# slimgroup/dfno

Measured on AMD Instinct MI355X. Metric: sec/batch, lower is better.
Workload: dtype fp32; 1 GPU; model=dfno-two-phase-3d, global_batch=1, t_in=1, t_out=30, width=20, num_blocks=4, parallelism=spatial-model-parallel 1x1x1x1x1x1, step=fwd+relative-Lp-loss+bwd+adam, spectral_weights=complex64

## Files before the change

### dfno_amd/csrc/bindings.cpp

```cpp
#include <torch/extension.h>

#include "kernels.h"

PYBIND11_MODULE(TORCH_EXTENSION_NAME, m) {
  m.doc() = "dfno_amd MI355X (gfx950) native kernels";
  m.def("channel_mix_fwd", &channel_mix_fwd,
        "fused channel linear + bias + gelu: returns (y, z)");
  m.def("channel_mix_fwd_t", &channel_mix_fwd_t,
        "transposed channel contraction (grad-x)");
  m.def("channel_mix_bwd_w", &channel_mix_bwd_w,
        "split-s grad-W (+grad-bias) reduction");
  m.def("linear_res_gelu_fwd", &linear_res_gelu_fwd,
        "fused y = gelu(W @ x + res): returns (y, z)");
  m.def("irfft_linear_res_gelu_fwd", &irfft_linear_res_gelu_fwd,
        "fused y = gelu(W @ x + pad_irfft(Yt)): returns (y, z)");
  m.def("gelu_fwd", &gelu_fwd, "exact gelu");
  m.def("gelu_bwd", &gelu_bwd, "gelu backward (gy, z) -> gz");
  m.def("add_gelu_fwd", &add_gelu_fwd, "fused residual add + gelu: returns (y, z)");
  m.def("proj_head_fwd", &proj_head_fwd, "fused linear->gelu->linear head");
  m.def("proj_head_bwd", &proj_head_bwd,
        "fused head backward: returns (gz3, gb3, gW4, gb4)");
  m.def("channel_mix_bwd_fused", &channel_mix_bwd_fused,
        "fused trunk mix backward: (gx, gW, gb, gz)");
  m.def("proj_head_bwd_fused", &proj_head_bwd_fused,
        "fully-fused flagship head backward: (gx, gW3, gb3, gW4, gb4)");
  m.def("lift_head_fwd", &lift_head_fwd, "fused time-lift + channel-lift + gelus");
  m.def("lift_head_bwd", &lift_head_bwd,
        "lift head backward: (gx, gW1, gb1, gW2, gb2)");
  m.def("adam_step_", &adam_step_, "fused Adam step (in-place)");
  m.def("adam_step_batch_", &adam_step_batch_, "fused Adam step over a tensor list");
  m.def("adam_step_batch_fp8_", &adam_step_batch_fp8_,
        "fused Adam step with in-kernel e4m3 requantization (delayed scaling)");
  m.def("dft_c2c", &dft_c2c, "truncated/padded complex DFT along a dim");
  m.def("dft_rfft_trunc", &dft_rfft_trunc, "real->kept-low-modes DFT (last dim)");
  m.def("dft_rfft_trunc_adj", &dft_rfft_trunc_adj, "adjoint of dft_rfft_trunc");
  m.def("dft_rfft_trunc_adj_acc", &dft_rfft_trunc_adj_acc,
        "adjoint of dft_rfft_trunc with fused accumulate addend");
  m.def("dft_pad_irfft", &dft_pad_irfft, "kept modes -> real inverse (last dim)");
  m.def("dft_pad_irfft_adj", &dft_pad_irfft_adj, "adjoint of dft_pad_irfft");
  m.def("dft_zt_fwd", &dft_zt_fwd,
        "fused truncated (z,t) 2-D analysis (real -> kept-mode c64)");
  m.def("dft_zt_inv", &dft_zt_inv,
        "fused padded (z,t) 2-D synthesis (kept-mode c64 -> real)");
  m.def("dft_pad_irfft_bf16", &dft_pad_irfft_bf16,
        "pad_irfft with bf16 output (bf16 compute config)");
  m.def("dft_rfft_trunc_adj_bf16", &dft_rfft_trunc_adj_bf16,
        "rfft_trunc adjoint with bf16 output");
  m.def("spectral_corner_fwd", &spectral_corner_fwd,
        "corner-block complex spectral contraction (accumulate into y box)");
  m.def("spectral_corner_bwd_x", &spectral_corner_bwd_x,
        "corner-block spectral contraction adjoint wrt x");
  m.def("spectral_corners_fwd", &spectral_corners_fwd,
        "all corner boxes in one launch");
  m.def("spectral_corners_bwd_x", &spectral_corners_bwd_x,
        "all corner boxes adjoint wrt x in one launch");
  m.def("spectral_corners_bwd_w", &spectral_corners_bwd_w,
// ... 20 lines not shown
```

### dfno_amd/csrc/epilogue.hip

```cpp

#include <hip/hip_runtime.h>
#include <torch/extension.h>
#include <ATen/hip/impl/HIPStreamMasqueradingAsCUDA.h>

#include <algorithm>
#include <vector>

#include "kernels.h"
#include "gelu_math.h"

namespace {

constexpr int kBlock = 256;

template <int IMAX, int VEC, int IT, int OT, int NT, int MT>
__global__ __launch_bounds__(kBlock) void irfft_mix_gelu_kernel(
    const float* __restrict__ x, const float* __restrict__ W,
    const float* __restrict__ Yt, const float* __restrict__ tw,
    float* __restrict__ y, float* __restrict__ z,
    int B, int I_, int O_, long L, int N_, int m_, int LT, float scale,
    bool write_z) {
  constexpr bool PIN = NT > 0;
  const int I = IT > 0 ? IT : I_;
  const int O = OT > 0 ? OT : O_;
  const int N = PIN ? NT : N_;
  const int m = PIN ? MT : m_;
  const int M2 = 2 * m;
  const long S = L * N;

  extern __shared__ __align__(16) char smem_raw[];
  float* Wl = reinterpret_cast<float*>(smem_raw);
  float* twl = Wl + (((size_t)O * I + 3) & ~(size_t)3);
  float* Yl = twl + (PIN ? 0 : (((size_t)N * M2 + 3) & ~(size_t)3));
  for (int k = threadIdx.x; k < O * I; k += kBlock) Wl[k] = W[k];
  if constexpr (!PIN)
    for (int k = threadIdx.x; k < N * M2; k += kBlock) twl[k] = tw[k];

  const int CPL = N / VEC;
  const int line = (int)threadIdx.x / CPL;
  const int t0 = ((int)threadIdx.x - line * CPL) * VEC;
  const bool role = line < LT;

  float twc[PIN ? VEC : 1][PIN ? MT : 1], tws[PIN ? VEC : 1][PIN ? MT : 1];
  if constexpr (PIN) {
#pragma unroll
    for (int v = 0; v < VEC; ++v) {
      const float* twj = tw + (size_t)(role ? t0 + v : 0) * M2;
#pragma unroll
      for (int k = 0; k < MT; ++k) {
        twc[v][k] = twj[2 * k];
        tws[v][k] = twj[2 * k + 1];
      }
    }
  }

  const long ntl = (L + LT - 1) / LT;
  for (long tile = blockIdx.x; tile < (long)B * ntl; tile += gridDim.x) {
    const int b = (int)(tile / ntl);
    const long l0 = (tile - (long)b * ntl) * LT;
    const int nl = (int)min((long)LT, L - l0);

    __syncthreads();
    const int run = nl * M2;
    if constexpr (PIN) {
      const int run4 = run / 4;
      for (int idx = threadIdx.x; idx < O * run4; idx += kBlock) {
        const int o = idx / run4;
        const int r4 = idx - o * run4;
        const int k = (r4 * 2) % MT;
        float4 v = *reinterpret_cast<const float4*>(
            Yt + (((long)b * O + o) * L + l0) * M2 + (long)r4 * 4);
        const bool e0 = (k == 0) || (2 * k == NT);
        const bool e1 = (2 * (k + 1) == NT);
        const float f0 = e0 ? scale : 2.0f * scale;
        const float f1 = e1 ? scale : 2.0f * scale;
        v.x = f0 * v.x; v.y = e0 ? 0.0f : f0 * v.y;
        v.z = f1 * v.z; v.w = e1 ? 0.0f : f1 * v.w;
        *reinterpret_cast<float4*>(Yl + (size_t)o * LT * M2 + (size_t)r4 * 4) = v;
      }
    } else {
      for (int idx = threadIdx.x; idx < O * run; idx += kBlock) {
        const int o = idx / run;
        const int r = idx - o * run;
        const int k = (r >> 1) % m;
        const bool edge = (k == 0) || (2 * k == N);
        const float f = edge ? scale : 2.0f * scale;
        float v = f * Yt[(((long)b * O + o) * L + l0) * M2 + r];
        if (edge && (r & 1)) v = 0.0f;
        Yl[(size_t)o * LT * M2 + r] = v;
      }
    }
    __syncthreads();

    if (!role || line >= nl) continue;

    const long s = (l0 + line) * N + t0;
    const float* xb = x + ((long)b * I) * S + s;
    float xr[IMAX][VEC];
#pragma unroll
    for (int i = 0; i < IMAX; ++i) {
      if (i < I) {
        if constexpr (VEC == 2) {
          const float2 v = *reinterpret_cast<const float2*>(xb + (long)i * S);
          xr[i][0] = v.x; xr[i][1] = v.y;
        } else {
#pragma unroll
          for (int v = 0; v < VEC; ++v) xr[i][v] = xb[(long)i * S + v];
        }
      }
    }

    float* yb = y + ((long)b * O) * S + s;
    float* zb = z + ((long)b * O) * S + s;
    const float* yline = Yl + (size_t)line * M2;
#pragma unroll 2
    for (int o = 0; o < (OT > 0 ? OT : 1 << 20); ++o) {
      if (OT == 0 && o >= O) break;
      float acc[VEC], syn[VEC];
#pragma unroll
      for (int v = 0; v < VEC; ++v) { acc[v] = 0.0f; syn[v] = 0.0f; }
#pragma unroll
// ... 1 lines not shown
        if (i < I) {
          const float wv = Wl[(size_t)o * I + i];
#pragma unroll
          for (int v = 0; v < VEC; ++v) acc[v] += wv * xr[i][v];
        }
      }
      const float* yo = yline + (size_t)o * LT * M2;
      if constexpr (PIN) {
        float yk[2 * MT];
#pragma unroll
        for (int q = 0; q < MT / 2; ++q) {
          const float4 v = *reinterpret_cast<const float4*>(yo + 4 * q);
          yk[4 * q] = v.x; yk[4 * q + 1] = v.y;
          yk[4 * q + 2] = v.z; yk[4 * q + 3] = v.w;
        }
#pragma unroll
        for (int k = 0; k < MT; ++k) {
#pragma unroll
          for (int v = 0; v < VEC; ++v)
            syn[v] += yk[2 * k] * twc[v][k] - yk[2 * k + 1] * tws[v][k];
        }
      } else {
        for (int k = 0; k < m; ++k) {
          const float yr_ = yo[2 * k], yi_ = yo[2 * k + 1];
#pragma unroll
          for (int v = 0; v < VEC; ++v) {
            const float* twj = twl + (size_t)(t0 + v) * M2;
            syn[v] += yr_ * twj[2 * k] - yi_ * twj[2 * k + 1];
          }
        }
      }
#pragma unroll
      for (int v = 0; v < VEC; ++v) acc[v] += syn[v];
      if constexpr (VEC == 2) {
        if (write_z)
          *reinterpret_cast<float2*>(zb + (long)o * S) =
              make_float2(acc[0], acc[1]);
        *reinterpret_cast<float2*>(yb + (long)o * S) =
            make_float2(dfno_gelu::gelu(acc[0]), dfno_gelu::gelu(acc[1]));
      } else {
#pragma unroll
        for (int v = 0; v < VEC; ++v) {
          if (write_z) zb[(long)o * S + v] = acc[v];
          yb[(long)o * S + v] = dfno_gelu::gelu(acc[v]);
        }
      }
    }
  }
}

}

std::vector<at::Tensor> irfft_linear_res_gelu_fwd(const at::Tensor& x,
                                                  const at::Tensor& W,
                                                  const at::Tensor& Yt,
                                                  int64_t n_out, bool need_z) {
  TORCH_CHECK(x.is_cuda() && x.is_contiguous() && x.scalar_type() == at::kFloat,
              "irfft_linear_res_gelu: x must be contiguous fp32 on GPU");
  TORCH_CHECK(W.is_cuda() && W.is_contiguous() && W.scalar_type() == at::kFloat,
              "irfft_linear_res_gelu: W must be contiguous fp32 on GPU");
  TORCH_CHECK(Yt.is_cuda() && Yt.is_contiguous() &&
              Yt.scalar_type() == at::kComplexFloat,
              "irfft_linear_res_gelu: Yt must be contiguous complex64 on GPU");
  TORCH_CHECK(x.dim() == 3 && W.dim() == 2 && Yt.dim() == 4,
              "irfft_linear_res_gelu: x [B,I,S], W [O,I], Yt [B,O,L,m]");
  const int B = (int)x.size(0), I = (int)x.size(1);
  const long S = x.size(2);
  const int O = (int)W.size(0);
  const long L = Yt.size(2);
  const int m = (int)Yt.size(3);
  const int N = (int)n_out;
  TORCH_CHECK((int)W.size(1) == I, "irfft_linear_res_gelu: W/I mismatch");
  TORCH_CHECK(Yt.size(0) == B && (int)Yt.size(1) == O && L * N == S,
              "irfft_linear_res_gelu: Yt shape mismatch");
  TORCH_CHECK(I >= 1 && I <= 32 && O >= 1 && O <= 64 && N >= 1 && N <= 64 &&
              m >= 1 && m <= 32 && m <= N / 2 + 1,
              "irfft_linear_res_gelu: needs I<=32, O<=64, N<=64, m<=min(32,N/2+1)");

  auto y = at::empty({B, O, S}, x.options());
  auto z = need_z ? at::empty({B, O, S}, x.options())
                  : at::empty({0}, x.options());
  if (x.numel() == 0) return {y, z};

  auto stream = at::hip::getCurrentHIPStreamMasqueradingAsCUDA().stream();
  auto tw = dfno_twiddle_table(N, m, false, x.options());
  const float scale = (float)(1.0 / (double)N);
  const float* xp = x.data_ptr<float>();
  const float* Wp = W.data_ptr<float>();
  const float* Yp = reinterpret_cast<const float*>(Yt.data_ptr());
  const float* twp = tw.data_ptr<float>();
  float* yp = y.data_ptr<float>();
  float* zp = need_z ? z.data_ptr<float>() : yp;

  auto pad4 = [](size_t n) { return (n + 3) & ~(size_t)3; };
  if (I == 20 && O == 20 && N == 30 && m == 8) {
    constexpr int LT = 17;
    const long ntiles = (long)B * ((L + LT - 1) / LT);
    const int grid = (int)std::min(ntiles, 256L * 8);
    const size_t smem = sizeof(float) * (pad4(400) + (size_t)20 * LT * 16);
    hipLaunchKernelGGL((irfft_mix_gelu_kernel<20, 2, 20, 20, 30, 8>),
                       dim3(grid), dim3(kBlock), smem, stream, xp, Wp, Yp, twp,
                       yp, zp, B, I, O, L, N, m, LT, scale, need_z);
  } else {
    int LT = kBlock / N;
    const size_t line_bytes = sizeof(float) * (size_t)O * 2 * m;
    LT = (int)std::max<size_t>(1, std::min<size_t>(LT, (32 * 1024) / line_bytes));
    const long ntiles = (long)B * ((L + LT - 1) / LT);
    const int grid = (int)std::min(ntiles, 256L * 8);
    const size_t smem = sizeof(float) * (pad4((size_t)O * I) +
                                         pad4((size_t)N * 2 * m) +
                                         (size_t)O * LT * 2 * m);
#define EPI_GENERIC(CAP)                                                       \
    hipLaunchKernelGGL((irfft_mix_gelu_kernel<CAP, 1, 0, 0, 0, 0>),            \
                       dim3(grid), dim3(kBlock), smem, stream, xp, Wp, Yp,     \
                       twp, yp, zp, B, I, O, L, N, m, LT, scale, need_z);
    if (I <= 8) { EPI_GENERIC(8) }
    else if (I <= 16) { EPI_GENERIC(16) }
    else if (I <= 24) { EPI_GENERIC(24) }
    else { EPI_GENERIC(32) }
#undef EPI_GENERIC
  }
  DFNO_CHECK_LAUNCH("irfft_linear_res_gelu");
  return {y, z};
}
```

### dfno_amd/csrc/kernels.h

```cpp
#pragma once

#include <torch/extension.h>
#define DFNO_CHECK_LAUNCH(what)                                            \
  do {                                                                     \
    hipError_t _e = hipGetLastError();                                     \
    TORCH_CHECK(_e == hipSuccess, what, " launch failed: ",                \
                hipGetErrorString(_e));                                    \
  } while (0)

#include <vector>

std::vector<at::Tensor> channel_mix_fwd(const at::Tensor& x, const at::Tensor& W,
                                        const at::Tensor& b, bool act);

at::Tensor channel_mix_fwd_t(const at::Tensor& gz, const at::Tensor& W);

std::vector<at::Tensor> linear_res_gelu_fwd(const at::Tensor& x, const at::Tensor& W,
                                            const at::Tensor& res);

std::vector<at::Tensor> irfft_linear_res_gelu_fwd(const at::Tensor& x,
                                                  const at::Tensor& W,
                                                  const at::Tensor& Yt,
                                                  int64_t n_out, bool need_z);

at::Tensor dfno_twiddle_table(int N, int m, bool analysis,
                              const at::TensorOptions& opt);

at::Tensor gelu_fwd(const at::Tensor& x);
at::Tensor gelu_bwd(const at::Tensor& gy, const at::Tensor& z);
std::vector<at::Tensor> add_gelu_fwd(const at::Tensor& a, const at::Tensor& b);

at::Tensor proj_head_fwd(const at::Tensor& x, const at::Tensor& W3,
                         const at::Tensor& b3, const at::Tensor& W4,
                         const at::Tensor& b4);
std::vector<at::Tensor> proj_head_bwd(const at::Tensor& gy, const at::Tensor& x,
                                      const at::Tensor& W3, const at::Tensor& b3,
                                      const at::Tensor& W4);
std::vector<at::Tensor> proj_head_bwd_fused(const at::Tensor& gy,
                                            const at::Tensor& x,
                                            const at::Tensor& W3,
                                            const at::Tensor& b3,
                                            const at::Tensor& W4);

std::vector<at::Tensor> channel_mix_bwd_w(const at::Tensor& gz, const at::Tensor& x,
                                          bool want_bias);

std::vector<at::Tensor> channel_mix_bwd_fused(const at::Tensor& gy,
                                              const at::Tensor& z,
                                              const at::Tensor& x,
                                              const at::Tensor& W,
                                              bool want_bias, bool want_gz);

at::Tensor lift_head_fwd(const at::Tensor& x, const at::Tensor& W1,
                         const at::Tensor& b1, const at::Tensor& W2,
                         const at::Tensor& b2);
std::vector<at::Tensor> lift_head_bwd(const at::Tensor& gy, const at::Tensor& x,
                                      const at::Tensor& W1, const at::Tensor& b1,
                                      const at::Tensor& W2, const at::Tensor& b2);

void adam_step_(at::Tensor& p, const at::Tensor& g, at::Tensor& m, at::Tensor& v,
                double lr, double beta1, double beta2, double eps,
                double weight_decay, int64_t step);
void adam_step_batch_(std::vector<at::Tensor> ps, std::vector<at::Tensor> gs,
                      std::vector<at::Tensor> ms, std::vector<at::Tensor> vs,
                      double lr, double beta1, double beta2, double eps,
                      double weight_decay, std::vector<int64_t> steps);
std::vector<int64_t> adam_step_batch_fp8_(
    std::vector<at::Tensor> ps, std::vector<at::Tensor> gs,
    std::vector<at::Tensor> ms, std::vector<at::Tensor> vs,
    double lr, double beta1, double beta2, double eps, double weight_decay,
    std::vector<int64_t> steps, std::vector<at::Tensor> qs,
    std::vector<at::Tensor> am_ins, std::vector<at::Tensor> am_outs);

at::Tensor dft_c2c(const at::Tensor& x, int64_t dim, int64_t n,
                   int64_t m_lo, int64_t m_hi, bool analysis, double scale);
at::Tensor dft_rfft_trunc(const at::Tensor& x, int64_t dim, int64_t m);
at::Tensor dft_rfft_trunc_adj(const at::Tensor& gy, int64_t dim, int64_t n);
at::Tensor dft_rfft_trunc_adj_acc(const at::Tensor& gy, int64_t dim, int64_t n,
                                  const at::Tensor& accum);
at::Tensor dft_pad_irfft(const at::Tensor& y, int64_t dim, int64_t n_out, int64_t m);
at::Tensor dft_pad_irfft_adj(const at::Tensor& gx, int64_t dim, int64_t m);
at::Tensor dft_zt_fwd(const at::Tensor& x, int64_t mz_lo, int64_t mz_hi,
                      int64_t mt, double scale, bool factors);
at::Tensor dft_zt_inv(const at::Tensor& y, int64_t Z, int64_t T,
// ... 45 lines not shown
```

### dfno_amd/csrc/mix_bwd.hip

```cpp

#include <hip/hip_runtime.h>
#include <hip/hip_bf16.h>
#include <torch/extension.h>
#include <ATen/hip/impl/HIPStreamMasqueradingAsCUDA.h>

#include "kernels.h"
#include "gelu_math.h"

namespace {

constexpr int kBlock = 256;

typedef float f32x4_mb __attribute__((ext_vector_type(4)));

__device__ __forceinline__ float mb_ld(const float* p) { return *p; }
__device__ __forceinline__ float mb_ld(const unsigned short* p) {
  return __uint_as_float(((unsigned int)*p) << 16);
}
__device__ __forceinline__ void mb_st(float* p, float v) { *p = v; }
__device__ __forceinline__ void mb_st(unsigned short* p, float v) {
  __hip_bfloat16 h = __float2bfloat16(v);
  *p = *reinterpret_cast<unsigned short*>(&h);
}

template <typename TIO, bool WG, int PH = 7, int TS = 64>
__global__ __launch_bounds__(kBlock, 4) void mix_bwd_fused_kernel(
    const TIO* __restrict__ gy, const TIO* __restrict__ z,
    const TIO* __restrict__ x, const float* __restrict__ W,
    TIO* __restrict__ gx, float* __restrict__ gW, float* __restrict__ gb,
    TIO* __restrict__ gzout, int B, long S) {
  constexpr int C = 20;
  constexpr int LD = TS + 4;
  extern __shared__ __align__(16) char smem_raw[];
  float* gzt = reinterpret_cast<float*>(smem_raw);
  float* xt = gzt + (size_t)C * LD;

  const int lane = (int)(threadIdx.x & 63);
  const int wave = (int)(threadIdx.x >> 6);
  const int l16 = lane & 15;
  const int kg = lane >> 4;

  f32x4_mb wacc;
  wacc = f32x4_mb{0.f, 0.f, 0.f, 0.f};

  const long stiles = (S + TS - 1) / TS;
  const long tend = (long)B * stiles;
  constexpr int NPF = (2 * C * TS + kBlock - 1) / kBlock;
  float pfa[NPF], pfb[NPF];
  auto prefetch = [&](long tt) {
    if (tt >= tend) return;
    const int b = (int)(tt / stiles);
    const long s0 = (tt % stiles) * TS;
    const int nv = (int)min((long)TS, S - s0);
#pragma unroll
    for (int q = 0; q < NPF; ++q) {
      const int r = (int)threadIdx.x + q * kBlock;
      const int row = r / TS;
      const int c = r - row * TS;
// ... 4 lines not shown
        } else {
          const long off = ((long)b * C + (row - C)) * S + s0 + c;
          a = mb_ld(gy + off);
          bb = mb_ld(z + off);
        }
      }
      pfa[q] = a;
      pfb[q] = bb;
    }
  };
  prefetch(blockIdx.x);

  for (long t = blockIdx.x; t < tend; t += gridDim.x) {
    const int b = (int)(t / stiles);
    const long s0 = (t % stiles) * TS;
    const int nv = (int)min((long)TS, S - s0);
    __syncthreads();
#pragma unroll
    for (int q = 0; q < NPF; ++q) {
      const int r = (int)threadIdx.x + q * kBlock;
      const int row = r / TS;
      const int c = r - row * TS;
      if (row < C) {
        xt[row * LD + c] = pfa[q];
      } else {
        const float gzv = pfa[q] * dfno_gelu::gelu_grad(pfb[q]);
        gzt[(row - C) * LD + c] = gzv;
        if (WG && c < nv)
          mb_st(gzout + ((long)b * C + (row - C)) * S + s0 + c, gzv);
      }
    }
    prefetch(t + gridDim.x);
    __syncthreads();
    if constexpr ((PH & 2) == 0 && (PH & 4) == 0) continue;
#pragma unroll
    for (int pp = 0; pp < ((PH & 2) ? (2 * (TS / 16)) / 4 : 0); ++pp) {
      const int p = wave + 4 * pp;
      const int mt = p / (TS / 16), nt = p % (TS / 16);
      const int m = mt * 16 + l16;
      const int n = nt * 16 + l16;
      const bool av = m < C;
      f32x4_mb c4 = {0.f, 0.f, 0.f, 0.f};
#pragma unroll
      for (int k = 0; k < C; k += 4) {
        const int ko = k + kg;
        const float a = av ? W[ko * C + m] : 0.f;
        const float bb = gzt[ko * LD + n];
        c4 = __builtin_amdgcn_mfma_f32_16x16x4f32(a, bb, c4, 0, 0, 0);
      }
      const long sc = s0 + nt * 16 + l16;
      if (sc < S) {
#pragma unroll
        for (int r = 0; r < 4; ++r) {
          const int i = mt * 16 + kg * 4 + r;
          if (i < C) mb_st(gx + ((long)b * C + i) * S + sc, c4[r]);
        }
      }
    }
    if constexpr ((PH & 4) != 0) {
      const int mt = wave >> 1, nt = wave & 1;
      const float* gr = gzt + (mt * 16 + l16) * LD;
      const int ncol = nt * 16 + l16;
      const float* xr = xt + ncol * LD;
      const bool av = (mt * 16 + l16) < C;
      const bool bx = ncol < C;
      const bool bones = ncol == C;
#pragma unroll 8
      for (int k = 0; k < TS; k += 4) {
        const float a = av ? gr[k + kg] : 0.f;
        const float bb = bx ? xr[k + kg] : (bones ? 1.f : 0.f);
        wacc = __builtin_amdgcn_mfma_f32_16x16x4f32(a, bb, wacc, 0, 0, 0);
      }
    }
  }

  {
    const int mt = wave >> 1, nt = wave & 1;
#pragma unroll
    for (int r = 0; r < 4; ++r) {
      const int o = mt * 16 + kg * 4 + r;
      const int n = nt * 16 + l16;
      const float v = wacc[r];
      if (o < C && v != 0.f) {
        if (n < C) atomicAdd(&gW[(size_t)o * C + n], v);
        else if (n == C && gb != nullptr) atomicAdd(&gb[o], v);
      }
    }
  }
}

}

std::vector<at::Tensor> channel_mix_bwd_fused(const at::Tensor& gy,
                                              const at::Tensor& z,
                                              const at::Tensor& x,
                                              const at::Tensor& W,
                                              bool want_bias, bool want_gz) {
  const bool bf16 = gy.scalar_type() == at::kBFloat16;
  TORCH_CHECK(gy.is_cuda() && gy.is_contiguous() && z.is_contiguous() &&
              x.is_contiguous() && W.is_contiguous() &&
              (bf16 || gy.scalar_type() == at::kFloat) &&
              x.scalar_type() == gy.scalar_type() &&
              z.scalar_type() == gy.scalar_type() &&
              W.scalar_type() == at::kFloat,
              "mix_bwd_fused: fp32/bf16 activations, fp32 W");
  int B = (int)x.size(0), I = (int)x.size(1);
  long S = x.size(2);
  int O = (int)W.size(0);
  TORCH_CHECK(I == 20 && O == 20, "mix_bwd_fused: trunk 20x20 only");
  TORCH_CHECK(gy.numel() == x.numel() && z.numel() == x.numel(),
              "mix_bwd_fused: shape mismatch");

  auto gx = at::empty({B, I, S}, x.options());
  auto fopt = x.options().dtype(at::kFloat);
  auto gW = at::zeros({O, I}, fopt);
  auto gb = want_bias ? at::zeros({O}, fopt) : at::empty({0}, fopt);
  auto gz = want_gz ? at::empty({B, O, S}, x.options())
                    : at::empty({0}, x.options());
  if (x.numel() == 0) return {gx, gW, gb, gz};

  auto stream = at::hip::getCurrentHIPStreamMasqueradingAsCUDA().stream();
  static const bool ts128 = []() {
    const char* e = getenv("DFNO_MIX_TS128");
    return e && e[0] == '1';
  }();
  const int TS = ts128 ? 128 : 64;
  size_t smem = sizeof(float) * 2 * 20 * (TS + 4);
  long stiles = (S + TS - 1) / TS;
  int grid = (int)std::min((long)B * stiles, 1024L);
  float* gbp = want_bias ? gb.data_ptr<float>() : nullptr;
  static const int ph = []() {
    const char* e = getenv("DFNO_MIX_PHASES");
    return e ? atoi(e) : 7;
  }();
#define MB_LAUNCH(TIO, WG, GZP) MB_LAUNCH_T(TIO, WG, GZP, 7, 64)
#define MB_LAUNCH_P(TIO, WG, GZP, PHV) MB_LAUNCH_T(TIO, WG, GZP, PHV, 64)
#define MB_LAUNCH_T(TIO, WG, GZP, PHV, TSV)                                  \
  hipLaunchKernelGGL((mix_bwd_fused_kernel<TIO, WG, PHV, TSV>), dim3(grid), \
                     dim3(kBlock), smem, stream,                             \
                     reinterpret_cast<const TIO*>(gy.data_ptr()),            \
                     reinterpret_cast<const TIO*>(z.data_ptr()),             \
                     reinterpret_cast<const TIO*>(x.data_ptr()),             \
                     W.data_ptr<float>(),                                    \
                     reinterpret_cast<TIO*>(gx.data_ptr()),                  \
                     gW.data_ptr<float>(), gbp, GZP, B, S)
  if (bf16) {
    auto gzp = want_gz ? reinterpret_cast<unsigned short*>(gz.data_ptr())
                       : nullptr;
    if (want_gz) MB_LAUNCH(unsigned short, true, gzp);
    else         MB_LAUNCH(unsigned short, false, nullptr);
  } else {
    auto gzp = want_gz ? reinterpret_cast<float*>(gz.data_ptr()) : nullptr;
    if (want_gz) {
      if (ts128) { MB_LAUNCH_T(float, true, gzp, 7, 128); }
      else if (ph == 1) { MB_LAUNCH_T(float, true, gzp, 1, 64); }
      else if (ph == 3) { MB_LAUNCH_T(float, true, gzp, 3, 64); }
      else if (ph == 5) { MB_LAUNCH_T(float, true, gzp, 5, 64); }
      else { MB_LAUNCH_T(float, true, gzp, 7, 64); }
    }
    else         MB_LAUNCH(float, false, nullptr);
  }
#undef MB_LAUNCH_T
#undef MB_LAUNCH_P
#undef MB_LAUNCH
  DFNO_CHECK_LAUNCH("mix_bwd_fused");
  return {gx, gW, gb, gz};
}
```

### dfno_amd/nn/block.py

```python

from __future__ import annotations

from typing import Dict, List, Tuple

import numpy as np
import torch
import torch.nn as nn

import os

from ..comm import (Repartition, _get_plan, repartition_complete,
                    repartition_issue)
from ..partition import Partition, compute_distribution_info
from ..ops import spectral_conv, add_gelu, linear_res_gelu, rfft_trunc, fft_trunc, pad_ifft, pad_irfft
from ..ops import irfft_linear_res_gelu, fused_epilogue_enabled, fused_epilogue_ok
from ..timing import comm_region
from .linear import BroadcastedLinear

__all__ = ["DistributedFNOBlock"]


class DistributedFNOBlock(nn.Module):

    def __init__(self, P_x: Partition, in_shape, modes,
# ... 234 lines not shown
        T = self.in_shape[-1]
        m = min(self.restrict_prefixes[self.dim_m[-1]], T // 2 + 1)
        if not fused_epilogue_ok(self.dtype, self.width, self.width, T, m):
            return False
        if len(self.dim_m) == 2:
            from ..ops.fft import zt_enabled
            if zt_enabled():
                return False
        return _get_plan(self.P_m, self.P_x, tuple(self.in_shape)).is_identity

    def _chunk_sizes(self, nch: int):
        w = self.width
        base, rem = divmod(w, nch)
        return [base + (1 if i < rem else 0) for i in range(nch)]

    @staticmethod
    def _with_c(shape, c):
        s = list(shape)
        s[1] = c
        return s

    def forward(self, x: torch.Tensor) -> torch.Tensor:
        self.dt_comm = 0.0

        x_in = x
        with comm_region() as r:
            W_res = self.linear.W_bcast(self.linear.W)
        self.linear.dt_comm = r.host_dt

        nch = self._pipeline_chunks()
        if nch > 1:
            y = self._forward_pipelined(x, nch)
        else:
            y, x_in, spectrum = self._forward_seq(x)
            if spectrum:
                T = self.in_shape[-1]
                return irfft_linear_res_gelu(
                    x_in, W_res, y, T // 2 + 1, T,
                    self.restrict_prefixes[self.dim_m[-1]])

        return linear_res_gelu(x_in, W_res, y)

    def _forward_seq(self, x: torch.Tensor):
        from ..ops.fft import (StashGradFn, new_stash_key, rfft_trunc_stash,
                               stash_fusable)

        saved: Dict[int, int] = {}
        x_orig = x
        with comm_region() as r:
            x = self.R1(x)
        self.dt_comm += r.host_dt

        x_epi = x_orig
        outermost = self.dim_m[-1]
        zt_stash = False
        if (x is x_orig and len(self.dim_m) == 2 and x.is_cuda
                and x.numel() > 0 and x.dtype == torch.float32
                and torch.is_grad_enabled() and x.requires_grad):
            from ..ops.fft import zt_enabled, zt_fwd, zt_native_ok
            z_dim = self.dim_m[0]
            mzl = self.restrict_prefixes[z_dim]
            mzh = self.restrict_suffixes.get(z_dim, 0)
            mt = self.restrict_prefixes[outermost]
            if zt_enabled() and zt_native_ok(x, mzl, mzh, mt):
                key = new_stash_key()
                saved[outermost] = x.shape[outermost] // 2 + 1
                saved[z_dim] = x.shape[z_dim]
                xm, tok = zt_fwd(x, mzl, mzh, mt, stash_key=key)
                x_epi = StashGradFn.apply(x_orig, tok, key)
                x = xm
                zt_stash = True
        if zt_stash:
            pass
        elif (x is x_orig
                and stash_fusable(x, outermost, self.restrict_prefixes[outermost])):
            key = new_stash_key()
            saved[outermost] = x.shape[outermost] // 2 + 1
            xm, tok = rfft_trunc_stash(x, outermost,
                                       self.restrict_prefixes[outermost], key)
            for dim in reversed(self.dim_m[:-1]):
                saved[dim] = xm.shape[dim]
                xm = fft_trunc(xm, dim, self.restrict_prefixes[dim],
                               self.restrict_suffixes.get(dim, 0))
            x_epi = StashGradFn.apply(x_orig, tok, key)
            x = xm
        else:
            x = self._fwd_m(x, saved)

        with comm_region() as r:
            x = self.R2(x)
        self.dt_comm += r.host_dt

        if x.numel() > 0:
            x = self._fwd_y(x, saved)
            y = spectral_conv(x, list(self.weights), self.corner_bounds,
                              self.width, fp8=self.spectral_fp8)
            y = self._inv_y(y, saved)
        else:
            y = x

        with comm_region() as r:
            y = self.R3(y)
        self.dt_comm += r.host_dt

        defer = (y.is_cuda and y.numel() > 0 and y.dtype == torch.complex64
                 and self._fuse_epilogue())
        y = self._inv_m(y, saved, defer_irfft=defer)
        if defer:
            return y, x_epi, True

        with comm_region() as r:
            y = self.R4(y)
        self.dt_comm += r.host_dt
        return y, x_epi, False

    def _forward_pipelined(self, x: torch.Tensor, nch: int) -> torch.Tensor:
        sizes = self._chunk_sizes(nch)
        saved: Dict[int, int] = {}

        xs = list(x.split(sizes, dim=1)) if x.numel() > 0 else [x] * nch

        with comm_region() as r:
            h1 = [repartition_issue(self.R1, xc.contiguous(),
                                    self._with_c(self.in_shape, c))
                  for xc, c in zip(xs, sizes)]
        self.dt_comm += r.host_dt

        h2 = []
        for h, c in zip(h1, sizes):
            with comm_region() as r:
                xc = repartition_complete(h)
            self.dt_comm += r.host_dt
            xc = self._fwd_m(xc, saved)
            with comm_region() as r:
                h2.append(repartition_issue(self.R2, xc,
                                            self._with_c(self.trunc_m_shape, c)))
            self.dt_comm += r.host_dt

        zs = []
        for h in h2:
            with comm_region() as r:
                xc = repartition_complete(h)
            self.dt_comm += r.host_dt
            zs.append(self._fwd_y(xc, saved))

        if all(z.numel() == 0 for z in zs):
            x = zs[0]
# ... 40 lines not shown
```

### dfno_amd/ops/epilogue.py

```python

from __future__ import annotations

import os

import torch

from .. import _ext
from .fft import pad_irfft
from .pointwise import linear_res_gelu

__all__ = ["irfft_linear_res_gelu", "fused_epilogue_enabled",
           "fused_epilogue_ok"]


def fused_epilogue_enabled() -> bool:
    return os.environ.get("DFNO_FUSED_EPILOGUE", "1") != "0"


def fused_epilogue_ok(dtype, I: int, O: int, n_out: int, m: int) -> bool:
    return (dtype == torch.float32 and 1 <= I <= 32 and 1 <= O <= 64
            and 1 <= n_out <= 64 and 1 <= m <= min(32, n_out // 2 + 1))


class _IrfftLinearResGeluFn(torch.autograd.Function):
    @staticmethod
    def forward(ctx, x, W, Yt, n_out):
        ext = _ext.get(required=True)
        B, I = x.shape[0], x.shape[1]
        O, m = W.shape[0], Yt.shape[-1]
        S = x.numel() // max(B * I, 1)
        x3 = x.reshape(B, I, S).contiguous()
        Y4 = Yt.reshape(B, O, S // n_out, m).contiguous()
        need_z = any(ctx.needs_input_grad[:3])
        Wc = W.contiguous()
        y3, z3 = ext.irfft_linear_res_gelu_fwd(x3, Wc, Y4, n_out, need_z)
        if need_z:
            ctx.save_for_backward(x3, Wc, z3)
        ctx.x_shape = tuple(x.shape)
        ctx.y_shape = tuple(Yt.shape)
        ctx.n_out = n_out
        return y3

    @staticmethod
    def backward(ctx, gy):
        ext = _ext.get(required=True)
        x3, W, z3 = ctx.saved_tensors
        gy = gy.contiguous()
        B, I, S = x3.shape
        O = W.shape[0]
        m = ctx.y_shape[-1]
        if I == 20 and O == 20:
            gx, gW, _, gz = ext.channel_mix_bwd_fused(gy, z3, x3, W,
                                                      False, True)
        else:
            gz = ext.gelu_bwd(gy, z3)
            gx = ext.channel_mix_fwd_t(gz, W)
            gW, _ = ext.channel_mix_bwd_w(gz, x3, False)
        gY = ext.dft_pad_irfft_adj(gz.reshape(B, O, S // ctx.n_out, ctx.n_out),
                                   3, m)
        return (gx.reshape(ctx.x_shape), gW.to(W.dtype),
                gY.reshape(ctx.y_shape), None)


def irfft_linear_res_gelu(x: torch.Tensor, W: torch.Tensor, Yt: torch.Tensor,
                          n_half: int, n_out: int, m: int) -> torch.Tensor:
    m = min(m, n_half)
    if (x.is_cuda and x.numel() > 0 and Yt.dtype == torch.complex64
            and Yt.shape[-1] == m and x.shape[-1] == n_out
            and fused_epilogue_ok(x.dtype, x.shape[1], W.shape[0], n_out, m)):
        out = _IrfftLinearResGeluFn.apply(x, W, Yt, n_out)
        shape = list(x.shape)
        shape[1] = W.shape[0]
        return out.reshape(shape)
    res = pad_irfft(Yt, -1, n_half, n_out, m, out_dtype=x.dtype)
    if res.dtype != x.dtype:
        res = res.to(x.dtype)
    return linear_res_gelu(x, W, res)
```

### dfno_amd/ops/fft.py

```python

from __future__ import annotations

import os

import torch

from .. import _ext
from ..dispatch import note_fallback

__all__ = ["rfft_trunc", "fft_trunc", "pad_ifft", "pad_irfft"]

_MAX_N = 256


def _native_ok(x: torch.Tensor, n: int, m: int, op: str) -> bool:
    if not x.is_cuda:
        return False
    ok = (n <= _MAX_N and m <= 32
          and x.dtype in (torch.float32, torch.complex64,
                          torch.float64, torch.complex128))
    if not ok:
        note_fallback(op, f"N={n} (cap {_MAX_N}) / m={m} (cap 32) / "
                      f"dtype {x.dtype} outside the native-DFT range")
    return ok
# ... 116 lines not shown


class StashGradFn(torch.autograd.Function):

    @staticmethod
    def forward(ctx, x, tok, key):
        ctx.key = key
        return x.view_as(x)

    @staticmethod
    def backward(ctx, g):
        _GRAD_STASH[ctx.key] = g.contiguous()
        return None, torch.empty(0, device=g.device), None


class _RfftTruncStashFn(torch.autograd.Function):
    @staticmethod
    def forward(ctx, x, dim, m, key):
        ext = _ext.get(required=True)
        ctx.dim, ctx.m, ctx.n, ctx.key = dim, m, x.shape[dim], key
        ctx.bf16 = x.dtype == torch.bfloat16
        y = ext.dft_rfft_trunc(x.contiguous(), dim, m)
        tok = torch.empty(0, device=x.device)
        return y, tok

    @staticmethod
    def backward(ctx, gy, gtok):
        ext = _ext.get(required=True)
        acc = _GRAD_STASH.pop(ctx.key, None)
        if acc is None:
            raise RuntimeError(
                "rfft stash: epilogue gradient missing (stash backward did "
                "not run before the rfft adjoint)")
        if ctx.bf16:
            gx = ext.dft_rfft_trunc_adj_bf16(gy.contiguous(), ctx.dim,
                                             ctx.n, acc)
        else:
            gx = ext.dft_rfft_trunc_adj_acc(gy.contiguous(), ctx.dim,
                                            ctx.n, acc)
        return gx, None, None, None


def rfft_trunc_stash(x, dim, m, key):
    d = dim % x.dim()
    m = min(m, x.shape[d] // 2 + 1)
    return _RfftTruncStashFn.apply(x, d, m, key)


def stash_fusable(x, dim, m) -> bool:
    d = dim % x.dim()
    m = min(m, x.shape[d] // 2 + 1)
    if not (d == x.dim() - 1 and x.is_cuda and x.numel() > 0
            and torch.is_grad_enabled() and x.requires_grad
            and x.shape[d] <= _MAX_N and m <= 32):
        return False
    if x.dtype == torch.bfloat16:
        return rfft_bf16_native_ok(x, d, m)
    return x.dtype in (torch.float32, torch.float64)



_ZT_EMPTY = {}


def _zt_empty(device):
    t = _ZT_EMPTY.get(device)
    if t is None:
# ... 129 lines not shown
```

Baseline: 20.14 ms.

## Fuse rfft adjoint with W^T·gz grad-x in the spectral epilogue backward

The epilogue backward now skips computing grad-x inside the fused mix-backward kernel and instead stashes (gz, W). The rfft-truncation adjoint then computes gx = W^T gz + rfft_adj(G) in one kernel, reusing the irfft-mix kernel template in an adjoint mode that loads a transposed W and skips the Hermitian scaling. This removes a separate grad-x write and read plus an accumulate pass. The cost is more coupling through the grad stash and a kernel variant that depends on the twiddle-table and transposition conventions being right.

```diff
diff --git a/dfno_amd/csrc/bindings.cpp b/dfno_amd/csrc/bindings.cpp
--- a/dfno_amd/csrc/bindings.cpp
+++ b/dfno_amd/csrc/bindings.cpp
@@ -14,6 +14,8 @@
         "fused y = gelu(W @ x + res): returns (y, z)");
   m.def("irfft_linear_res_gelu_fwd", &irfft_linear_res_gelu_fwd,
         "fused y = gelu(W @ x + pad_irfft(Yt)): returns (y, z)");
+  m.def("rfft_adj_mix", &rfft_adj_mix,
+        "fused gx = W^T @ gz + rfft_trunc_adj(G, n)");
   m.def("gelu_fwd", &gelu_fwd, "exact gelu");
   m.def("gelu_bwd", &gelu_bwd, "gelu backward (gy, z) -> gz");
   m.def("add_gelu_fwd", &add_gelu_fwd, "fused residual add + gelu: returns (y, z)");
@@ -21,7 +23,9 @@
   m.def("proj_head_bwd", &proj_head_bwd,
         "fused head backward: returns (gz3, gb3, gW4, gb4)");
   m.def("channel_mix_bwd_fused", &channel_mix_bwd_fused,
-        "fused trunk mix backward: (gx, gW, gb, gz)");
+        "fused trunk mix backward: (gx, gW, gb, gz)",
+        py::arg("gy"), py::arg("z"), py::arg("x"), py::arg("W"),
+        py::arg("want_bias"), py::arg("want_gz"), py::arg("want_gx") = true);
   m.def("proj_head_bwd_fused", &proj_head_bwd_fused,
         "fully-fused flagship head backward: (gx, gW3, gb3, gW4, gb4)");
   m.def("lift_head_fwd", &lift_head_fwd, "fused time-lift + channel-lift + gelus");
diff --git a/dfno_amd/csrc/epilogue.hip b/dfno_amd/csrc/epilogue.hip
--- a/dfno_amd/csrc/epilogue.hip
+++ b/dfno_amd/csrc/epilogue.hip
@@ -13,7 +13,7 @@
 
 constexpr int kBlock = 256;
 
-template <int IMAX, int VEC, int IT, int OT, int NT, int MT>
+template <int IMAX, int VEC, int IT, int OT, int NT, int MT, bool ADJ = false>
 __global__ __launch_bounds__(kBlock) void irfft_mix_gelu_kernel(
     const float* __restrict__ x, const float* __restrict__ W,
     const float* __restrict__ Yt, const float* __restrict__ tw,
@@ -32,7 +32,14 @@
   float* Wl = reinterpret_cast<float*>(smem_raw);
   float* twl = Wl + (((size_t)O * I + 3) & ~(size_t)3);
   float* Yl = twl + (PIN ? 0 : (((size_t)N * M2 + 3) & ~(size_t)3));
-  for (int k = threadIdx.x; k < O * I; k += kBlock) Wl[k] = W[k];
+  if constexpr (ADJ) {
+    for (int k = threadIdx.x; k < O * I; k += kBlock) {
+      const int o = k / I;
+      Wl[k] = W[(size_t)(k - o * I) * O + o];
+    }
+  } else {
+    for (int k = threadIdx.x; k < O * I; k += kBlock) Wl[k] = W[k];
+  }
   if constexpr (!PIN)
     for (int k = threadIdx.x; k < N * M2; k += kBlock) twl[k] = tw[k];
 
@@ -67,26 +74,31 @@
       for (int idx = threadIdx.x; idx < O * run4; idx += kBlock) {
         const int o = idx / run4;
         const int r4 = idx - o * run4;
-        const int k = (r4 * 2) % MT;
         float4 v = *reinterpret_cast<const float4*>(
             Yt + (((long)b * O + o) * L + l0) * M2 + (long)r4 * 4);
-        const bool e0 = (k == 0) || (2 * k == NT);
-        const bool e1 = (2 * (k + 1) == NT);
-        const float f0 = e0 ? scale : 2.0f * scale;
-        const float f1 = e1 ? scale : 2.0f * scale;
-        v.x = f0 * v.x; v.y = e0 ? 0.0f : f0 * v.y;
-        v.z = f1 * v.z; v.w = e1 ? 0.0f : f1 * v.w;
+        if constexpr (!ADJ) {
+          const int k = (r4 * 2) % MT;
+          const bool e0 = (k == 0) || (2 * k == NT);
+          const bool e1 = (2 * (k + 1) == NT);
+          const float f0 = e0 ? scale : 2.0f * scale;
+          const float f1 = e1 ? scale : 2.0f * scale;
+          v.x = f0 * v.x; v.y = e0 ? 0.0f : f0 * v.y;
+          v.z = f1 * v.z; v.w = e1 ? 0.0f : f1 * v.w;
+        }
         *reinterpret_cast<float4*>(Yl + (size_t)o * LT * M2 + (size_t)r4 * 4) = v;
       }
     } else {
       for (int idx = threadIdx.x; idx < O * run; idx += kBlock) {
         const int o = idx / run;
         const int r = idx - o * run;
-        const int k = (r >> 1) % m;
-        const bool edge = (k == 0) || (2 * k == N);
-        const float f = edge ? scale : 2.0f * scale;
-        float v = f * Yt[(((long)b * O + o) * L + l0) * M2 + r];
-        if (edge && (r & 1)) v = 0.0f;
+        float v = Yt[(((long)b * O + o) * L + l0) * M2 + r];
+        if constexpr (!ADJ) {
+          const int k = (r >> 1) % m;
+          const bool edge = (k == 0) || (2 * k == N);
+          const float f = edge ? scale : 2.0f * scale;
+          v = f * v;
+          if (edge && (r & 1)) v = 0.0f;
+        }
         Yl[(size_t)o * LT * M2 + r] = v;
       }
     }
@@ -154,7 +166,15 @@
       }
 #pragma unroll
       for (int v = 0; v < VEC; ++v) acc[v] += syn[v];
-      if constexpr (VEC == 2) {
+      if constexpr (ADJ) {
+        if constexpr (VEC == 2) {
+          *reinterpret_cast<float2*>(yb + (long)o * S) =
+              make_float2(acc[0], acc[1]);
+        } else {
+#pragma unroll
+          for (int v = 0; v < VEC; ++v) yb[(long)o * S + v] = acc[v];
+        }
+      } else if constexpr (VEC == 2) {
         if (write_z)
           *reinterpret_cast<float2*>(zb + (long)o * S) =
               make_float2(acc[0], acc[1]);
@@ -168,6 +188,41 @@
         }
       }
     }
+  }
+}
+
+template <bool ADJ>
+void launch_irfft_mix(const float* xp, const float* Wp, const float* Yp,
+                      const float* twp, float* yp, float* zp, int B, int I,
+                      int O, long L, int N, int m, float scale, bool write_z,
+                      hipStream_t stream) {
+  auto pad4 = [](size_t n) { return (n + 3) & ~(size_t)3; };
+  if (I == 20 && O == 20 && N == 30 && m == 8) {
+    constexpr int LT = 17;
+    const long ntiles = (long)B * ((L + LT - 1) / LT);
+    const int grid = (int)std::min(ntiles, 256L * 8);
+    const size_t smem = sizeof(float) * (pad4(400) + (size_t)20 * LT * 16);
+    hipLaunchKernelGGL((irfft_mix_gelu_kernel<20, 2, 20, 20, 30, 8, ADJ>),
+                       dim3(grid), dim3(kBlock), smem, stream, xp, Wp, Yp, twp,
+                       yp, zp, B, I, O, L, N, m, LT, scale, write_z);
+  } else {
+    int LT = kBlock / N;
+    const size_t line_bytes = sizeof(float) * (size_t)O * 2 * m;
+    LT = (int)std::max<size_t>(1, std::min<size_t>(LT, (32 * 1024) / line_bytes));
+    const long ntiles = (long)B * ((L + LT - 1) / LT);
+    const int grid = (int)std::min(ntiles, 256L * 8);
+    const size_t smem = sizeof(float) * (pad4((size_t)O * I) +
+                                         pad4((size_t)N * 2 * m) +
+                                         (size_t)O * LT * 2 * m);
+#define EPI_GENERIC(CAP)                                                       \
+    hipLaunchKernelGGL((irfft_mix_gelu_kernel<CAP, 1, 0, 0, 0, 0, ADJ>),       \
+                       dim3(grid), dim3(kBlock), smem, stream, xp, Wp, Yp,     \
+                       twp, yp, zp, B, I, O, L, N, m, LT, scale, write_z);
+    if (I <= 8) { EPI_GENERIC(8) }
+    else if (I <= 16) { EPI_GENERIC(16) }
+    else if (I <= 24) { EPI_GENERIC(24) }
+    else { EPI_GENERIC(32) }
+#undef EPI_GENERIC
   }
 }
 
@@ -207,41 +262,51 @@
   auto stream = at::hip::getCurrentHIPStreamMasqueradingAsCUDA().stream();
   auto tw = dfno_twiddle_table(N, m, false, x.options());
   const float scale = (float)(1.0 / (double)N);
-  const float* xp = x.data_ptr<float>();
-  const float* Wp = W.data_ptr<float>();
-  const float* Yp = reinterpret_cast<const float*>(Yt.data_ptr());
-  const float* twp = tw.data_ptr<float>();
   float* yp = y.data_ptr<float>();
   float* zp = need_z ? z.data_ptr<float>() : yp;
-
-  auto pad4 = [](size_t n) { return (n + 3) & ~(size_t)3; };
-  if (I == 20 && O == 20 && N == 30 && m == 8) {
-    constexpr int LT = 17;
-    const long ntiles = (long)B * ((L + LT - 1) / LT);
-    const int grid = (int)std::min(ntiles, 256L * 8);
-    const size_t smem = sizeof(float) * (pad4(400) + (size_t)20 * LT * 16);
-    hipLaunchKernelGGL((irfft_mix_gelu_kernel<20, 2, 20, 20, 30, 8>),
-                       dim3(grid), dim3(kBlock), smem, stream, xp, Wp, Yp, twp,
-                       yp, zp, B, I, O, L, N, m, LT, scale, need_z);
-  } else {
-    int LT = kBlock / N;
-    const size_t line_bytes = sizeof(float) * (size_t)O * 2 * m;
-    LT = (int)std::max<size_t>(1, std::min<size_t>(LT, (32 * 1024) / line_bytes));
-    const long ntiles = (long)B * ((L + LT - 1) / LT);
-    const int grid = (int)std::min(ntiles, 256L * 8);
-    const size_t smem = sizeof(float) * (pad4((size_t)O * I) +
-                                         pad4((size_t)N * 2 * m) +
-                                         (size_t)O * LT * 2 * m);
-#define EPI_GENERIC(CAP)                                                       \
-    hipLaunchKernelGGL((irfft_mix_gelu_kernel<CAP, 1, 0, 0, 0, 0>),            \
-                       dim3(grid), dim3(kBlock), smem, stream, xp, Wp, Yp,     \
-                       twp, yp, zp, B, I, O, L, N, m, LT, scale, need_z);
-    if (I <= 8) { EPI_GENERIC(8) }
-    else if (I <= 16) { EPI_GENERIC(16) }
-    else if (I <= 24) { EPI_GENERIC(24) }
-    else { EPI_GENERIC(32) }
-#undef EPI_GENERIC
-  }
+  launch_irfft_mix<false>(x.data_ptr<float>(), W.data_ptr<float>(),
+                          reinterpret_cast<const float*>(Yt.data_ptr()),
+                          tw.data_ptr<float>(), yp, zp, B, I, O, L, N, m,
+                          scale, need_z, stream);
   DFNO_CHECK_LAUNCH("irfft_linear_res_gelu");
   return {y, z};
 }
+
+at::Tensor rfft_adj_mix(const at::Tensor& gz, const at::Tensor& W,
+                        const at::Tensor& G, int64_t n) {
+  TORCH_CHECK(gz.is_cuda() && gz.is_contiguous() &&
+              gz.scalar_type() == at::kFloat,
+              "rfft_adj_mix: gz must be contiguous fp32 on GPU");
+  TORCH_CHECK(W.is_cuda() && W.is_contiguous() && W.scalar_type() == at::kFloat,
+              "rfft_adj_mix: W must be contiguous fp32 on GPU");
+  TORCH_CHECK(G.is_cuda() && G.is_contiguous() &&
+              G.scalar_type() == at::kComplexFloat,
+              "rfft_adj_mix: G must be contiguous complex64 on GPU");
+  TORCH_CHECK(gz.dim() == 3 && W.dim() == 2 && G.dim() == 4,
+              "rfft_adj_mix: gz [B,O,S], W [O,I], G [B,I,L,m]");
+  const int B = (int)gz.size(0), O = (int)gz.size(1);
+  const long S = gz.size(2);
+  const int I = (int)W.size(1);
+  const long L = G.size(2);
+  const int m = (int)G.size(3);
+  const int N = (int)n;
+  TORCH_CHECK((int)W.size(0) == O, "rfft_adj_mix: W/O mismatch");
+  TORCH_CHECK(G.size(0) == B && (int)G.size(1) == I && L * N == S,
+              "rfft_adj_mix: G shape mismatch");
+  TORCH_CHECK(O >= 1 && O <= 32 && I >= 1 && I <= 64 && N >= 1 && N <= 64 &&
+              m >= 1 && m <= 32 && m <= N / 2 + 1,
+              "rfft_adj_mix: needs O<=32, I<=64, N<=64, m<=min(32,N/2+1)");
+
+  auto gx = at::empty({B, I, S}, gz.options());
+  if (gz.numel() == 0) return gx;
+
+  auto stream = at::hip::getCurrentHIPStreamMasqueradingAsCUDA().stream();
+  auto tw = dfno_twiddle_table(N, m, false, gz.options());
+  float* gp = gx.data_ptr<float>();
+  launch_irfft_mix<true>(gz.data_ptr<float>(), W.data_ptr<float>(),
+                         reinterpret_cast<const float*>(G.data_ptr()),
+                         tw.data_ptr<float>(), gp, gp, B, O, I, L,
+                         N, m, 1.0f, false, stream);
+  DFNO_CHECK_LAUNCH("rfft_adj_mix");
+  return gx;
+}
diff --git a/dfno_amd/csrc/kernels.h b/dfno_amd/csrc/kernels.h
--- a/dfno_amd/csrc/kernels.h
+++ b/dfno_amd/csrc/kernels.h
@@ -22,6 +22,9 @@
                                                   const at::Tensor& W,
                                                   const at::Tensor& Yt,
                                                   int64_t n_out, bool need_z);
+
+at::Tensor rfft_adj_mix(const at::Tensor& gz, const at::Tensor& W,
+                        const at::Tensor& G, int64_t n);
 
 at::Tensor dfno_twiddle_table(int N, int m, bool analysis,
                               const at::TensorOptions& opt);
@@ -49,7 +52,8 @@
                                               const at::Tensor& z,
                                               const at::Tensor& x,
                                               const at::Tensor& W,
-                                              bool want_bias, bool want_gz);
+                                              bool want_bias, bool want_gz,
+                                              bool want_gx = true);
 
 at::Tensor lift_head_fwd(const at::Tensor& x, const at::Tensor& W1,
                          const at::Tensor& b1, const at::Tensor& W2,
diff --git a/dfno_amd/csrc/mix_bwd.hip b/dfno_amd/csrc/mix_bwd.hip
--- a/dfno_amd/csrc/mix_bwd.hip
+++ b/dfno_amd/csrc/mix_bwd.hip
@@ -23,7 +23,7 @@
   *p = *reinterpret_cast<unsigned short*>(&h);
 }
 
-template <typename TIO, bool WG, int PH = 7, int TS = 64>
+template <typename TIO, bool WG, int PH = 7, int TS = 64, bool WX = true>
 __global__ __launch_bounds__(kBlock, 4) void mix_bwd_fused_kernel(
     const TIO* __restrict__ gy, const TIO* __restrict__ z,
     const TIO* __restrict__ x, const float* __restrict__ W,
@@ -94,9 +94,10 @@
     }
     prefetch(t + gridDim.x);
     __syncthreads();
-    if constexpr ((PH & 2) == 0 && (PH & 4) == 0) continue;
-#pragma unroll
-    for (int pp = 0; pp < ((PH & 2) ? (2 * (TS / 16)) / 4 : 0); ++pp) {
+    constexpr bool kPhaseA = WX && (PH & 2) != 0;
+    if constexpr (!kPhaseA && (PH & 4) == 0) continue;
+#pragma unroll
+    for (int pp = 0; pp < (kPhaseA ? (2 * (TS / 16)) / 4 : 0); ++pp) {
       const int p = wave + 4 * pp;
       const int mt = p / (TS / 16), nt = p % (TS / 16);
       const int m = mt * 16 + l16;
@@ -157,7 +158,8 @@
                                               const at::Tensor& z,
                                               const at::Tensor& x,
                                               const at::Tensor& W,
-                                              bool want_bias, bool want_gz) {
+                                              bool want_bias, bool want_gz,
+                                              bool want_gx) {
   const bool bf16 = gy.scalar_type() == at::kBFloat16;
   TORCH_CHECK(gy.is_cuda() && gy.is_contiguous() && z.is_contiguous() &&
               x.is_contiguous() && W.is_contiguous() &&
@@ -173,7 +175,11 @@
   TORCH_CHECK(gy.numel() == x.numel() && z.numel() == x.numel(),
               "mix_bwd_fused: shape mismatch");
 
-  auto gx = at::empty({B, I, S}, x.options());
+  TORCH_CHECK(want_gx || want_gz,
+              "mix_bwd_fused: want_gx=false needs want_gz (grad-x is then "
+              "the caller's W^T gz)");
+  auto gx = want_gx ? at::empty({B, I, S}, x.options())
+                    : at::empty({0}, x.options());
   auto fopt = x.options().dtype(at::kFloat);
   auto gW = at::zeros({O, I}, fopt);
   auto gb = want_bias ? at::zeros({O}, fopt) : at::empty({0}, fopt);
@@ -206,7 +212,21 @@
                      W.data_ptr<float>(),                                    \
                      reinterpret_cast<TIO*>(gx.data_ptr()),                  \
                      gW.data_ptr<float>(), gbp, GZP, B, S)
-  if (bf16) {
+#define MB_LAUNCH_NOGX(TIO, GZP)                                             \
+  hipLaunchKernelGGL((mix_bwd_fused_kernel<TIO, true, 7, 64, false>),       \
+                     dim3(grid), dim3(kBlock), smem, stream,                 \
+                     reinterpret_cast<const TIO*>(gy.data_ptr()),            \
+                     reinterpret_cast<const TIO*>(z.data_ptr()),             \
+                     reinterpret_cast<const TIO*>(x.data_ptr()),             \
+                     W.data_ptr<float>(), static_cast<TIO*>(nullptr),        \
+                     gW.data_ptr<float>(), gbp, GZP, B, S)
+  if (!want_gx) {
+    if (bf16)
+      MB_LAUNCH_NOGX(unsigned short,
+                     reinterpret_cast<unsigned short*>(gz.data_ptr()));
+    else
+      MB_LAUNCH_NOGX(float, reinterpret_cast<float*>(gz.data_ptr()));
+  } else if (bf16) {
     auto gzp = want_gz ? reinterpret_cast<unsigned short*>(gz.data_ptr())
                        : nullptr;
     if (want_gz) MB_LAUNCH(unsigned short, true, gzp);
@@ -222,6 +242,7 @@
     }
     else         MB_LAUNCH(float, false, nullptr);
   }
+#undef MB_LAUNCH_NOGX
 #undef MB_LAUNCH_T
 #undef MB_LAUNCH_P
 #undef MB_LAUNCH
diff --git a/dfno_amd/nn/block.py b/dfno_amd/nn/block.py
--- a/dfno_amd/nn/block.py
+++ b/dfno_amd/nn/block.py
@@ -290,12 +290,12 @@
         if nch > 1:
             y = self._forward_pipelined(x, nch)
         else:
-            y, x_in, spectrum = self._forward_seq(x)
+            y, x_in, spectrum, stash = self._forward_seq(x)
             if spectrum:
                 T = self.in_shape[-1]
                 return irfft_linear_res_gelu(
                     x_in, W_res, y, T // 2 + 1, T,
-                    self.restrict_prefixes[self.dim_m[-1]])
+                    self.restrict_prefixes[self.dim_m[-1]], stash=stash)
 
         return linear_res_gelu(x_in, W_res, y)
 
@@ -310,6 +310,7 @@
         self.dt_comm += r.host_dt
 
         x_epi = x_orig
+        stash = None
         outermost = self.dim_m[-1]
         zt_stash = False
         if (x is x_orig and len(self.dim_m) == 2 and x.is_cuda
@@ -340,7 +341,7 @@
                 saved[dim] = xm.shape[dim]
                 xm = fft_trunc(xm, dim, self.restrict_prefixes[dim],
                                self.restrict_suffixes.get(dim, 0))
-            x_epi = StashGradFn.apply(x_orig, tok, key)
+            stash = (key, tok)
             x = xm
         else:
             x = self._fwd_m(x, saved)
@@ -365,12 +366,14 @@
                  and self._fuse_epilogue())
         y = self._inv_m(y, saved, defer_irfft=defer)
         if defer:
-            return y, x_epi, True
+            return y, x_epi, True, stash
+        if stash is not None:
+            x_epi = StashGradFn.apply(x_orig, stash[1], stash[0])
 
         with comm_region() as r:
             y = self.R4(y)
         self.dt_comm += r.host_dt
-        return y, x_epi, False
+        return y, x_epi, False, None
 
     def _forward_pipelined(self, x: torch.Tensor, nch: int) -> torch.Tensor:
         sizes = self._chunk_sizes(nch)
diff --git a/dfno_amd/ops/epilogue.py b/dfno_amd/ops/epilogue.py
--- a/dfno_amd/ops/epilogue.py
+++ b/dfno_amd/ops/epilogue.py
@@ -6,11 +6,11 @@
 import torch
 
 from .. import _ext
-from .fft import pad_irfft
+from .fft import _GRAD_STASH, StashGradFn, pad_irfft
 from .pointwise import linear_res_gelu
 
 __all__ = ["irfft_linear_res_gelu", "fused_epilogue_enabled",
-           "fused_epilogue_ok"]
+           "fused_epilogue_ok", "fused_rfft_adj_enabled", "rfft_adj_mix_ok"]
 
 
 def fused_epilogue_enabled() -> bool:
@@ -22,16 +22,26 @@
             and 1 <= n_out <= 64 and 1 <= m <= min(32, n_out // 2 + 1))
 
 
+def fused_rfft_adj_enabled() -> bool:
+    return os.environ.get("DFNO_FUSED_RFFT_ADJ", "1") != "0"
+
+
+def rfft_adj_mix_ok(dtype, I: int, O: int, n: int, m: int) -> bool:
+    return (dtype == torch.float32 and 1 <= O <= 32 and 1 <= I <= 64
+            and 1 <= n <= 64 and 1 <= m <= min(32, n // 2 + 1))
+
+
 class _IrfftLinearResGeluFn(torch.autograd.Function):
+
     @staticmethod
-    def forward(ctx, x, W, Yt, n_out):
+    def forward(ctx, x, W, Yt, n_out, key=None, tok=None):
         ext = _ext.get(required=True)
         B, I = x.shape[0], x.shape[1]
         O, m = W.shape[0], Yt.shape[-1]
         S = x.numel() // max(B * I, 1)
         x3 = x.reshape(B, I, S).contiguous()
         Y4 = Yt.reshape(B, O, S // n_out, m).contiguous()
-        need_z = any(ctx.needs_input_grad[:3])
+        need_z = any(ctx.needs_input_grad[:3]) or key is not None
         Wc = W.contiguous()
         y3, z3 = ext.irfft_linear_res_gelu_fwd(x3, Wc, Y4, n_out, need_z)
         if need_z:
@@ -39,6 +49,7 @@
         ctx.x_shape = tuple(x.shape)
         ctx.y_shape = tuple(Yt.shape)
         ctx.n_out = n_out
+        ctx.key = key
         return y3
 
     @staticmethod
@@ -49,6 +60,18 @@
         B, I, S = x3.shape
         O = W.shape[0]
         m = ctx.y_shape[-1]
+        if ctx.key is not None:
+            if I == 20 and O == 20:
+                _, gW, _, gz = ext.channel_mix_bwd_fused(gy, z3, x3, W,
+                                                         False, True, False)
+            else:
+                gz = ext.gelu_bwd(gy, z3)
+                gW, _ = ext.channel_mix_bwd_w(gz, x3, False)
+            _GRAD_STASH[ctx.key] = (gz, W)
+            gY = ext.dft_pad_irfft_adj(
+                gz.reshape(B, O, S // ctx.n_out, ctx.n_out), 3, m)
+            return (None, gW.to(W.dtype), gY.reshape(ctx.y_shape), None,
+                    None, torch.empty(0, device=gy.device))
         if I == 20 and O == 20:
             gx, gW, _, gz = ext.channel_mix_bwd_fused(gy, z3, x3, W,
                                                       False, True)
@@ -59,15 +82,27 @@
         gY = ext.dft_pad_irfft_adj(gz.reshape(B, O, S // ctx.n_out, ctx.n_out),
                                    3, m)
         return (gx.reshape(ctx.x_shape), gW.to(W.dtype),
-                gY.reshape(ctx.y_shape), None)
+                gY.reshape(ctx.y_shape), None, None, None)
 
 
 def irfft_linear_res_gelu(x: torch.Tensor, W: torch.Tensor, Yt: torch.Tensor,
-                          n_half: int, n_out: int, m: int) -> torch.Tensor:
+                          n_half: int, n_out: int, m: int,
+                          stash=None) -> torch.Tensor:
     m = min(m, n_half)
-    if (x.is_cuda and x.numel() > 0 and Yt.dtype == torch.complex64
-            and Yt.shape[-1] == m and x.shape[-1] == n_out
-            and fused_epilogue_ok(x.dtype, x.shape[1], W.shape[0], n_out, m)):
+    fused = (x.is_cuda and x.numel() > 0 and Yt.dtype == torch.complex64
+             and Yt.shape[-1] == m and x.shape[-1] == n_out
+             and fused_epilogue_ok(x.dtype, x.shape[1], W.shape[0], n_out, m))
+    if stash is not None:
+        key, tok = stash
+        if (fused and fused_rfft_adj_enabled()
+                and rfft_adj_mix_ok(x.dtype, x.shape[1], W.shape[0], n_out, m)):
+            out = _IrfftLinearResGeluFn.apply(x.detach(), W, Yt, n_out,
+                                              key, tok)
+            shape = list(x.shape)
+            shape[1] = W.shape[0]
+            return out.reshape(shape)
+        x = StashGradFn.apply(x, tok, key)
+    if fused:
         out = _IrfftLinearResGeluFn.apply(x, W, Yt, n_out)
         shape = list(x.shape)
         shape[1] = W.shape[0]
diff --git a/dfno_amd/ops/fft.py b/dfno_amd/ops/fft.py
--- a/dfno_amd/ops/fft.py
+++ b/dfno_amd/ops/fft.py
@@ -172,7 +172,15 @@
             raise RuntimeError(
                 "rfft stash: epilogue gradient missing (stash backward did "
                 "not run before the rfft adjoint)")
-        if ctx.bf16:
+        if isinstance(acc, tuple):
+            gz, W = acc
+            G = gy.contiguous()
+            shape = list(G.shape)
+            shape[-1] = ctx.n
+            gx = ext.rfft_adj_mix(
+                gz, W, G.reshape(gz.shape[0], W.shape[1], -1, ctx.m), ctx.n)
+            gx = gx.reshape(shape)
+        elif ctx.bf16:
             gx = ext.dft_rfft_trunc_adj_bf16(gy.contiguous(), ctx.dim,
                                              ctx.n, acc)
         else:
```

Result: faster. 18.55 ms, median of 6 (-7.9%).
